# psaegert/bcnf

Hardware: AMD Instinct MI355X
Metric: NLL-training samples/sec + log_prob max-abs-err vs ref, trajectory_FC_small (higher is better)
Workload: dtype f32; 1 GPU; trajectory_FC_small NLL training step (configs[1]); batch_per_gpu=4096, global_batch=4096, parallelism=dp1, hip_graph=True, n_blocks=32, n_conditions=80

## Files before the change

bcnf_amd/csrc/bcnf_stack.hip:

```cpp
#include "bcnf_device.h"
#include "../../include/bcnf_amd.h"

#include <math.h>
#include <stdlib.h>
#include <string.h>

#include <algorithm>
#include <mutex>
#include <utility>
#include <vector>


#ifdef BCNF_PHASE_STAMPS
#define BCNF_STAMPS 1
#else
#define BCNF_STAMPS 0
#endif

namespace {

constexpr int NC16_MAX = 16;
constexpr int TILE = 256;
__host__ __device__ constexpr int tile_slot(int r, int q) { return 4 * r + ((q + (r >> 1)) & 3); }
__host__ __device__ constexpr int tile_ix(int s, int r) { return 4 * tile_slot(r, s & 3) + (s >> 2); }
// ... 514 lines not shown
      r[i] = g4[idx < n4 ? idx : 0];
    }
  }
  __device__ __forceinline__ void store(float* __restrict__ s) const { store_t(s, (int)threadIdx.x); }
  __device__ __forceinline__ void load_t(const float* __restrict__ g, int n, int t) {
    const floatx4* g4 = reinterpret_cast<const floatx4*>(g);
    const int n4 = n >> 2;
#pragma unroll
    for (int i = 0; i < N; ++i) {
      const int idx = t + i * BCNF_WG;
      r[i] = g4[idx < n4 ? idx : 0];
    }
  }
  __device__ __forceinline__ void store_t(float* __restrict__ s, int t) const {
    floatx4* s4 = reinterpret_cast<floatx4*>(s);
#pragma unroll
    for (int i = 0; i < N; ++i) s4[t + i * BCNF_WG] = r[i];
  }
};

constexpr int KC = 128;
constexpr int KCP = KC + 4;
constexpr int BNS = 80;
__host__ __device__ constexpr int bstride16(int n) { return n + ((16 - (n & 31)) & 31); }

template <bool VEC>
__device__ __forceinline__ void load_rows64(const float* __restrict__ M, long long nrows, int ncols, long long ld,
                                            long long r0, int c0, floatx4* reg, int ones = -1) {
#pragma unroll
  for (int e = 0; e < 8; ++e) {
    const int i4 = threadIdx.x + 256 * e, row = i4 >> 5, col = c0 + (i4 & 31) * 4;
    const long long r = r0 + row < nrows ? r0 + row : nrows - 1;
    if (VEC) {
      const floatx4 v = *reinterpret_cast<const floatx4*>(M + r * ld + (col < ncols ? col : 0));
#pragma unroll
      for (int q = 0; q < 4; ++q) reg[e][q] = (r0 + row < nrows && col + q < ncols) ? v[q] : 0.f;
    } else {
#pragma unroll
      for (int q = 0; q < 4; ++q) {
        const int cq = col + q;
        const float v = M[r * ld + (cq < ncols ? cq : ncols - 1)];
        reg[e][q] = (r0 + row < nrows && cq < ncols) ? v : 0.f;
      }
    }
    if (ones >= 0) {
#pragma unroll
      for (int q = 0; q < 4; ++q)
        if (col + q == ones && r0 + row < nrows) reg[e][q] = 1.f;
    }
  }
}

template <bool VEC>
__global__ __launch_bounds__(BCNF_WG) void k_hp(BcnfLayout L, const float* __restrict__ pk,
                                                const float* __restrict__ h, long long R, float* __restrict__ hp) {
  extern __shared__ __attribute__((aligned(16))) float smem[];
  float* As = smem;
  float* Bs = smem + 64 * KCP;
  const int tid = threadIdx.x, wave = tid >> 6, l = tid & 63, lr = l & 15, lq = l >> 4;
  const long long b0 = (long long)blockIdx.x * 64;
  const int n0 = blockIdx.y * 64;
  const int Cp = L.Cp, NKp = L.NKp;
  const float* w1c = pk + L.w1c_off;
  floatx4 ra[8], rb[8];
  auto load = [&](int c0) {
    load_rows64<VEC>(h, R, L.C, L.ldh, b0, c0, ra);
#pragma unroll
    for (int e = 0; e < 8; ++e) {
      const int i4 = tid + 256 * e, row = c0 + (i4 >> 4), col = n0 + (i4 & 15) * 4;
      const floatx4 v = *reinterpret_cast<const floatx4*>(w1c + (long long)(row < Cp ? row : Cp - 1) * NKp + col);
      rb[e] = v * (row < Cp ? 1.f : 0.f);
    }
  };
  auto store = [&]() {
#pragma unroll
    for (int e = 0; e < 8; ++e) {
      const int i4 = tid + 256 * e;
      *reinterpret_cast<floatx4*>(As + (i4 >> 5) * KCP + (i4 & 31) * 4) = ra[e];
      *reinterpret_cast<floatx4*>(Bs + (i4 >> 4) * BNS + (i4 & 15) * 4) = rb[e];
    }
  };
  floatx4 acc[4];
#pragma unroll
  for (int u = 0; u < 4; ++u) acc[u] = floatx4{0.f, 0.f, 0.f, 0.f};
  load(0);
  float b1v[4];
#pragma unroll
  for (int u = 0; u < 4; ++u) b1v[u] = pk[L.b1c_off + n0 + 16 * u + lr];
  for (int c0 = 0; c0 < Cp; c0 += KC) {
    store();
    __syncthreads();
    if (c0 + KC < Cp) load(c0 + KC);
    const int ks = (Cp - c0 < KC ? Cp - c0 : KC) >> 2;
    for (int t0 = 0; t0 < ks; t0 += 4) {
      float a[4], bv[4][4];
#pragma unroll
      for (int t = 0; t < 4; ++t) {
        a[t] = As[(16 * wave + lr) * KCP + 4 * (t0 + t) + lq];
#pragma unroll
        for (int u = 0; u < 4; ++u) bv[t][u] = Bs[(4 * (t0 + t) + lq) * BNS + 16 * u + lr];
      }
#pragma unroll
      for (int t = 0; t < 4; ++t)
#pragma unroll
        for (int u = 0; u < 4; ++u) acc[u] = mfma4(a[t], bv[t][u], acc[u]);
    }
// ... 32 lines not shown
      ra[e] = v * (k < L.nb ? 1.f : 0.f);
    }
#pragma unroll
    for (int e = 0; e < 2; ++e) {
      const int i4 = tid + 256 * e, kj = kj0 + (i4 >> 2);
      const floatx4 v = *reinterpret_cast<const floatx4*>(w1r + (long long)(kj < K ? kj : K - 1) * Cp + (i4 & 3) * 4);
      rb[e] = v * (kj < K ? 1.f : 0.f);
    }
  };
  auto store = [&]() {
#pragma unroll
    for (int e = 0; e < 8; ++e) *reinterpret_cast<floatx4*>(As + arow * KCP + 16 * e + aj4) = ra[e];
#pragma unroll
    for (int e = 0; e < 2; ++e) *reinterpret_cast<floatx4*>(Bs + (tid + 256 * e) * 4) = rb[e];
  };
  floatx4 acc = {0.f, 0.f, 0.f, 0.f}, acc1 = {0.f, 0.f, 0.f, 0.f};
  load(0);
  for (int kj0 = 0; kj0 < K; kj0 += KC) {
    store();
    __syncthreads();
    if (kj0 + KC < K) load(kj0 + KC);
    const int ks = (K - kj0 < KC ? K - kj0 : KC) >> 2;
    for (int t0 = 0; t0 < ks; t0 += 4) {
      float a[4], bv[4];
#pragma unroll
      for (int t = 0; t < 4; ++t) {
        a[t] = As[(16 * wave + lr) * KCP + 4 * (t0 + t) + lq];
        bv[t] = Bs[(4 * (t0 + t) + lq) * 16 + lr];
      }
      acc = mfma4(a[0], bv[0], acc);
      acc1 = mfma4(a[1], bv[1], acc1);
      acc = mfma4(a[2], bv[2], acc);
      acc1 = mfma4(a[3], bv[3], acc1);
    }
    __syncthreads();
  }
  acc += acc1;
  const int col = 16 * n + lr;
  if (col < L.C) {
#pragma unroll
    for (int i = 0; i < 4; ++i) {
      const long long r = b0 + 16 * wave + 4 * lq + i;
      if (r < B) dh[r * L.C + col] = acc[i];
    }
  }
}

__global__ __launch_bounds__(BCNF_WG) void k_dh(BcnfLayout L, const float* __restrict__ pk,
                                                const float* __restrict__ d1, long long B, float* __restrict__ dh) {
  extern __shared__ __attribute__((aligned(16))) float smem[];
  dh_body(L, pk, d1, B, dh, blockIdx.x, blockIdx.y, smem);
}

template <bool VEC, int BPW = 4>
__device__ __forceinline__ void dw1h_body(const BcnfLayout& L, const float* __restrict__ d1, const float* __restrict__ h,
                                          long long B, int rows_per_split, float* __restrict__ work, int bx, int by,
                                          float* __restrict__ smem, int ones = -1) {
  const int hs = bstride16(L.Cp);
  float* As = smem;
  float* Bs = smem + 16 * BPW * KCP;
  const int tid = threadIdx.x, wave = tid >> 6, l = tid & 63, lr = l & 15, lq = l >> 4;
  const int k0 = bx * BPW, s = by;
  const long long m0 = (long long)s * rows_per_split;
  long long m1 = m0 + rows_per_split;
  if (m1 > B) m1 = B;
  const int NC16 = L.Cp >> 4;
  {
    const int row = tid >> 1, j8 = (tid & 1) * 8;
    const long long b = m0 + row;
    const bool ok = b < m1;
    const long long bb = ok ? b : m1 - 1;
    floatx4 va[2 * BPW];
#pragma unroll
    for (int kk = 0; kk < BPW; ++kk) {
      const int k = k0 + kk < L.nb ? k0 + kk : L.nb - 1;
      const floatx4* src = reinterpret_cast<const floatx4*>(d1 + ((long long)k * B + bb) * 16 + j8);
      va[2 * kk] = src[0];
      va[2 * kk + 1] = src[1];
    }
    floatx4 rv[2][8];
#pragma unroll
    for (int half = 0; half < 2; ++half) load_rows64<VEC>(h, m1, L.C, L.ldh, m0 + 64 * half, 0, rv[half], ones);
#pragma unroll
    for (int kk = 0; kk < BPW; ++kk) {
      const float m = (ok && k0 + kk < L.nb) ? 1.f : 0.f;
      const floatx4 v0 = va[2 * kk] * m, v1 = va[2 * kk + 1] * m;
#pragma unroll
      for (int q = 0; q < 4; ++q) {
        As[(kk * 16 + j8 + q) * KCP + row] = v0[q];
        As[(kk * 16 + j8 + 4 + q) * KCP + row] = v1[q];
      }
    }
#pragma unroll
    for (int half = 0; half < 2; ++half) {
#pragma unroll
      for (int e = 0; e < 8; ++e) {
        const int i4 = tid + 256 * e, r = 64 * half + (i4 >> 5), col = (i4 & 31) * 4;
        if (col < L.Cp) *reinterpret_cast<floatx4*>(Bs + r * hs + col) = rv[half][e];
      }
    }
    for (int c0 = KC; c0 < L.Cp; c0 += KC) {
#pragma unroll
      for (int half = 0; half < 2; ++half) {
        load_rows64<VEC>(h, m1, L.C, L.ldh, m0 + 64 * half, c0, rv[half], ones);
#pragma unroll
        for (int e = 0; e < 8; ++e) {
          const int i4 = tid + 256 * e, r = 64 * half + (i4 >> 5), col = c0 + (i4 & 31) * 4;
          if (col < L.Cp) *reinterpret_cast<floatx4*>(Bs + r * hs + col) = rv[half][e];
        }
      }
    }
  }
  __syncthreads();
  const int kw = BPW == 4 ? wave : wave >> 1;
  const int k = k0 + kw;
  const int nh = BPW == 4 ? NC16 : (NC16 + 1) >> 1;
  const int n_lo = BPW == 4 ? 0 : (wave & 1) * nh, n_hi = min(NC16, n_lo + nh);
  float* o = work + (((long long)s * L.nb + (k < L.nb ? k : 0)) * 16) * L.Cp;
  for (int n = n_lo; n < n_hi; ++n) {
    floatx4 acc = {0.f, 0.f, 0.f, 0.f}, acc1 = {0.f, 0.f, 0.f, 0.f};
    for (int t0 = 0; t0 < KC / 4; t0 += 8) {
      float a[8], bv[8];
#pragma unroll
      for (int t = 0; t < 8; ++t) {
        a[t] = As[(16 * kw + lr) * KCP + 4 * (t0 + t) + lq];
        bv[t] = Bs[(4 * (t0 + t) + lq) * hs + 16 * n + lr];
      }
#pragma unroll
      for (int t = 0; t < 8; t += 2) {
        acc = mfma4(a[t], bv[t], acc);
        acc1 = mfma4(a[t + 1], bv[t + 1], acc1);
      }
    }
    acc += acc1;
    if (k < L.nb) {
#pragma unroll
      for (int i = 0; i < 4; ++i) o[(long long)(4 * lq + i) * L.Cp + 16 * n + lr] = acc[i];
    }
  }
}

template <bool VEC>
__global__ __launch_bounds__(BCNF_WG) void k_dw1h(BcnfLayout L, const float* __restrict__ d1,
                                                  const float* __restrict__ h, long long B, int rows_per_split,
                                                  float* __restrict__ work) {
  extern __shared__ __attribute__((aligned(16))) float smem[];
  dw1h_body<VEC>(L, d1, h, B, rows_per_split, work, blockIdx.x, blockIdx.y, smem);
}

size_t hp_lds_bytes() { return sizeof(float) * (size_t)(64 * KCP + KC * BNS); }
size_t dh_lds_bytes() { return sizeof(float) * (size_t)(64 * KCP + KC * 16); }
size_t dw1h_lds_bytes(const BcnfLayout& L, int bpw = 4) {
  return sizeof(float) * (size_t)(16 * bpw * KCP + KC * bstride16(L.Cp));
}

template <bool VEC>
__global__ __launch_bounds__(BCNF_WG) void k_fold_splitk(BcnfLayout F, const float* __restrict__ d1,
                                                         const float* __restrict__ x, long long B, int rows_per_split,
                                                         float* __restrict__ work, int gx_dw, int ones,
                                                         FoldAdamArgs A) {
  extern __shared__ __attribute__((aligned(16))) float smem[];
  if (A.on && blockIdx.x == gridDim.x - 1) {
    if (threadIdx.x == 0) adam_scalars_publish(A);
    return;
  }
  dw1h_body<VEC, 2>(F, d1, x, B, rows_per_split, work, blockIdx.x % gx_dw, blockIdx.x / gx_dw, smem, ones);
}

__global__ __launch_bounds__(BCNF_WG) void k_dw1h_reduce(BcnfLayout L, const float* __restrict__ work, int splits,
                                                         float* __restrict__ dparams) {
  const long long per = 16LL * L.Cp, total = (long long)L.nb * per;
  const long long i = (long long)blockIdx.x * BCNF_WG + threadIdx.x;
  if (i >= total) return;
  const int k = (int)(i / per);
  const int rem = (int)(i - (long long)k * per);
  const int j = rem / L.Cp, c = rem - j * L.Cp;
  if (j >= L.H[1] || c >= L.C) return;
  float acc = 0.f;
  int s = 0;
  for (; s + 8 <= splits; s += 8) {
    float v[8];
#pragma unroll
    for (int t = 0; t < 8; ++t) v[t] = work[(long long)(s + t) * total + i];
#pragma unroll
    for (int t = 0; t < 8; ++t) acc += v[t];
  }
  for (; s < splits; ++s) acc += work[(long long)s * total + i];
  dparams[coupling_base(L, k) + L.lin_w[1] + j * L.lin_in[1] + L.Da + c] = acc;
}

__device__ __forceinline__ void gx_reduce_body(long long total, const float* __restrict__ work, int splits,
                                               float* __restrict__ gx, long long i) {
  if (i >= total) return;
  float acc = 0.f;
  int s = 0;
  for (; s + 16 <= splits; s += 16) {
    float v[16];
#pragma unroll
    for (int t = 0; t < 16; ++t) v[t] = work[(long long)(s + t) * total + i];
#pragma unroll
    for (int t = 0; t < 16; ++t) acc += v[t];
  }
  for (; s < splits; ++s) acc += work[(long long)s * total + i];
  gx[i] = acc;
}

__device__ __forceinline__ int c0_of_finish(int bx, int nct) { return (bx % nct) * 16; }

constexpr int FIN_KC = 512;
constexpr int FIN_SMEM = 2 * FIN_KC * 16;

__device__ __forceinline__ void tile16_accum(const float* __restrict__ As, const float* __restrict__ Bs, int kn,
                                             floatx4 (&acc)[4]) {
  const int lane = threadIdx.x & 63, ks = lane & 15, rb = lane >> 4, cb = threadIdx.x >> 6;
#pragma unroll 4
  for (int k = ks; k < kn; k += 16) {
    const floatx4 a = *reinterpret_cast<const floatx4*>(As + k * 16 + 4 * rb);
    const floatx4 b = *reinterpret_cast<const floatx4*>(Bs + k * 16 + 4 * cb);
#pragma unroll
    for (int r = 0; r < 4; ++r)
#pragma unroll
      for (int c = 0; c < 4; ++c) acc[r][c] = fmaf(a[r], b[c], acc[r][c]);
  }
}

__device__ __forceinline__ float tile16_reduce(float* __restrict__ red, const floatx4 (&acc)[4]) {
  const int lane = threadIdx.x & 63, ks = lane & 15, rb = lane >> 4, cb = threadIdx.x >> 6;
  __syncthreads();
#pragma unroll
  for (int r = 0; r < 4; ++r)
#pragma unroll
    for (int c = 0; c < 4; ++c) red[ks * 256 + (4 * rb + r) * 16 + 4 * cb + c] = acc[r][c];
  __syncthreads();
  float v = 0.f;
#pragma unroll
  for (int q = 0; q < 16; ++q) v += red[q * 256 + threadIdx.x];
  return v;
}

__global__ __launch_bounds__(BCNF_WG) void k_fold_finish(BcnfLayout L, const float* __restrict__ pk,
                                                         const float* __restrict__ gx, const float* __restrict__ wf,
                                                         const float* __restrict__ bf, int X,
                                                         float* __restrict__ dparams, float* __restrict__ dwf,
                                                         float* __restrict__ dbf, FoldAdamArgs A) {
  extern __shared__ __attribute__((aligned(16))) float smem[];
  float* As = smem;
  float* Bs = smem + FIN_KC * 16;
  const int Xp = fold_xp(X), tid = threadIdx.x, nct = L.Cp >> 4;
  floatx4 acc[4];
#pragma unroll
  for (int q = 0; q < 4; ++q) acc[q] = floatx4{0.f, 0.f, 0.f, 0.f};
  const bool adam = A.on && !(A.guard && A.guard[BCNF_GUARD_HALTED]);
  AdamScalars as{};
  const bool keeper = adam && blockIdx.x == 0 && tid == 0;
  const bool logger = keeper && A.log_values && A.log_history;
  long long log_row = 0;
  float step0 = 0.f, log_v[3];
// ... 1410 lines not shown
      }
      gya = an_sa * dxa;
      gyb = an_sb * dxb;
      PHS(1)
      __syncthreads();
      PHS(2)
    }
    if (dy && valid) {
      if (j < Da) dy[b * D + j] = gya;
      if (j < Db) dy[b * D + Da + j] = gyb;
    }
  }
#if BCNF_STAMPS
  if (blockIdx.x == 0 && (threadIdx.x == 0 || threadIdx.x == BCNF_WG))
    for (int i = 0; i < 4; ++i) g_phase[(helper ? 4 : 0) + i] = ph_acc[i];
#endif
#undef PHS
  if (loss_out && blockIdx.x == 0) {
    __syncthreads();
    nll_finalize<BWD_WG>(nll_part, (int)gridDim.x, B, loss_out, rng_w, guard, dT);
  }
}

template <int N>
__device__ __forceinline__ int lpick(const int (&a)[N], int i) {
  int r = a[0];
#pragma unroll
  for (int t = 1; t < N; ++t) r = (i == t) ? a[t] : r;
  return r;
}

__device__ __forceinline__ long long slab_to_canonical(const BcnfLayout& L, int m, int o) {
  const int NH = L.NH, NW = NH + 2;
  const int cb = m * L.blk_stride + ((m < L.nb - 1) ? L.an_size : 0);
  if (o < NW * 256) {
    const int c = o >> 8, e = o & 255, lane = e >> 2;
    const int row = 4 * (lane >> 4) + (e & 3), col = lane & 15;
    const int l = c < NH ? c + 1 : NH + 1;
    const int nrows = c < NH ? lpick(L.H, l) : L.Db, ncols = (l == 1) ? L.Da : lpick(L.H, l - 1);
    if (row >= nrows || col >= ncols) return -1;
    const int row0 = (c == NH + 1) ? L.Db : 0;
    return (long long)cb + lpick(L.lin_w, l) + (row0 + row) * lpick(L.lin_in, l) + col;
  }
  const int o2 = o - NW * 256, c = o2 >> 4, r = o2 & 15;
  if (c < NH) return r < lpick(L.H, c + 1) ? (long long)cb + lpick(L.lin_b, c + 1) + r : -1;
  if (c < NH + 2) return r < L.Db ? (long long)cb + lpick(L.lin_b, NH + 1) + ((c == NH + 1) ? L.Db : 0) + r : -1;
  const int a = c - NH - 2;
  if (a >= 4 || !L.act_norm || m >= L.nb - 1 || r >= ((a < 2) ? L.Da : L.Db)) return -1;
  return (long long)m * L.blk_stride + ((a & 1) ? L.D : 0) + ((a < 2) ? 0 : L.Da) + r;
}

constexpr int RED_G = 8, RED_O4 = 32, RED_T = 16;

__device__ __forceinline__ void reduce_body(const BcnfLayout& L, const float* __restrict__ slab, long long stride,
                                            int nwg, float* __restrict__ out, int bx, float* __restrict__ smem,
                                            const FoldAdamArgs* A = nullptr, const AdamScalars* as = nullptr) {
  floatx4 (*part)[RED_O4] = reinterpret_cast<floatx4 (*)[RED_O4]>(smem);
  const int g = threadIdx.x / RED_O4, o4 = threadIdx.x % RED_O4;
  const long long i = ((long long)bx * RED_O4 + o4) * 4;
  const bool live = i < stride;
  const long long ic = live ? i : 0;
  const int m = (int)(ic / L.sblk), o = (int)(ic - (long long)m * L.sblk);
  long long ci[4];
  float ap[4], am[4], av[4];
#pragma unroll
  for (int e = 0; e < 4; ++e) {
    ci[e] = slab_to_canonical(L, m, o + e);
    if (A && g == 0) {
      const long long c = ci[e] >= 0 ? ci[e] : 0;
      ap[e] = A->p[0][c];
      am[e] = A->m[0][c];
      av[e] = A->v[0][c];
    }
  }
  floatx4 acc = {0.f, 0.f, 0.f, 0.f};
  int w = g;
  for (; w + RED_G * (RED_T - 1) < nwg; w += RED_G * RED_T) {
    floatx4 v[RED_T];
#pragma unroll
    for (int t = 0; t < RED_T; ++t)
      v[t] = *reinterpret_cast<const floatx4*>(slab + (long long)(w + RED_G * t) * stride + ic);
#pragma unroll
    for (int t = 0; t < RED_T; ++t) acc += v[t];
  }
  for (; w < nwg; w += RED_G) acc += *reinterpret_cast<const floatx4*>(slab + (long long)w * stride + ic);
  part[g][o4] = acc;
  __syncthreads();
  if (g != 0 || !live) return;
  floatx4 tot = part[0][o4];
#pragma unroll
  for (int q = 1; q < RED_G; ++q) tot += part[q][o4];
#pragma unroll
  for (int e = 0; e < 4; ++e) {
    if (ci[e] < 0) continue;
    out[ci[e]] = tot[e];
    if (A) {
      adam_elem(ap[e], tot[e], am[e], av[e], *as);
      A->p[0][ci[e]] = ap[e];
      A->m[0][ci[e]] = am[e];
      A->v[0][ci[e]] = av[e];
    }
  }
}

struct TailGrid {
  int n_dh, gx_dh;
  int n_red;
  int gx_dw;
  int ones;
};

template <bool VEC>
__global__ __launch_bounds__(BCNF_WG) void k_bwd_tail(BcnfLayout L, BcnfLayout Lw, TailGrid G, const float* __restrict__ pk,
                                                      const float* __restrict__ d1, const float* __restrict__ h,
                                                      long long B, float* __restrict__ dh,
                                                      const float* __restrict__ slab, long long stride, int nwg,
                                                      float* __restrict__ dparams, int rows_per_split,
                                                      float* __restrict__ work) {
  extern __shared__ __attribute__((aligned(16))) float smem[];
  int i = blockIdx.x;
  if (i < G.n_dh) {
    dh_body(L, pk, d1, B, dh, i % G.gx_dh, i / G.gx_dh, smem);
    return;
  }
  i -= G.n_dh;
  if (i < G.n_red) {
    reduce_body(L, slab, stride, nwg, dparams, i, smem);
    return;
  }
  i -= G.n_red;
  dw1h_body<VEC>(Lw, d1, h, B, rows_per_split, work, i % G.gx_dw, i / G.gx_dw, smem, G.ones);
}

__global__ __launch_bounds__(BCNF_WG) void k_red_gx(BcnfLayout L, long long total, const float* __restrict__ work,
                                                    int splits, float* __restrict__ gx, int n_gx,
                                                    const float* __restrict__ slab, long long stride, int nwg,
                                                    float* __restrict__ dparams, FoldAdamArgs A) {
  __shared__ __attribute__((aligned(16))) float smem[RED_G * RED_O4 * 4];
  const int bx = blockIdx.x;
  if (bx < n_gx) {
    gx_reduce_body(total, work, splits, gx, (long long)bx * BCNF_WG + threadIdx.x);
    return;
  }
  if (A.on && !(A.guard && A.guard[BCNF_GUARD_HALTED])) {
    const AdamScalars as = adam_scalars_of(A, A.asc[0], A.asc[1]);
    reduce_body(L, slab, stride, nwg, dparams, bx - n_gx, smem, &A, &as);
    return;
  }
  reduce_body(L, slab, stride, nwg, dparams, bx - n_gx, smem);
}

__global__ __launch_bounds__(BCNF_WG) void k_fill_lds(float value) {
  extern __shared__ __attribute__((aligned(16))) float smem[];
  for (int i = threadIdx.x; i < (int)(LDS_MAX / 16); i += BCNF_WG)
    reinterpret_cast<floatx4*>(smem)[i] = floatx4{value, value, value, value};
  __syncthreads();
}

int check_launch() { return bcnf_rt::launched(); }



std::mutex g_attr_mu;
const void* g_attr_fn[256];
size_t g_attr_lds[256];
int g_attr_n = 0;

template <typename K>
int launch_lds(K kernel, size_t& lds) {
  if (lds > LDS_MAX) return BCNF_ERR_UNSUPPORTED;
  const void* fn = reinterpret_cast<const void*>(kernel);
  std::lock_guard<std::mutex> lk(g_attr_mu);
  for (int i = 0; i < g_attr_n; ++i)
    if (g_attr_fn[i] == fn && g_attr_lds[i] >= lds) return BCNF_OK;
  const hipError_t e = hipFuncSetAttribute(fn, hipFuncAttributeMaxDynamicSharedMemorySize, (int)lds);
  if (e != hipSuccess) return bcnf_rt::hip_status(e);
  int slot = -1;
  for (int i = 0; i < g_attr_n; ++i)
    if (g_attr_fn[i] == fn) slot = i;
  if (slot < 0 && g_attr_n < 256) slot = g_attr_n++;
  if (slot >= 0) {
    g_attr_fn[slot] = fn;
    g_attr_lds[slot] = lds;
  }
  return BCNF_OK;
}

template <int NH>
bool layout_matches(const BcnfLayout& L) {
  return L.rf_b1 == RecF<NH>::B1 && L.rf_w1 == RecF<NH>::W1 && L.rf_hid == RecF<NH>::HID && L.rf_t == RecF<NH>::T &&
         L.rf_s == RecF<NH>::S && L.rf_q == RecF<NH>::Q && L.RF >= RecF<NH>::USED && L.rb_w1t == RecB<NH>::W1T &&
         L.rb_hid == RecB<NH>::HID && L.rb_tt == RecB<NH>::TT && L.rb_st == RecB<NH>::ST && L.rb_qt == RecB<NH>::QT &&
         L.rb_an == RecB<NH>::AN && L.RB >= RecB<NH>::USED;
}

struct NllOut {
  float* part = nullptr;
};

bool vec_rows(const BcnfLayout& L, const float* h) { return L.ldh % 4 == 0 && ((uintptr_t)h & 15) == 0; }

int launch_hp(const BcnfLayout& L, const float* pk, const float* h, long long R, float* hp, hipStream_t st) {
// ... 208 lines not shown
}

int bcnf_stack_forward(const BcnfStackDesc* desc, const void* packed, const float* y, const float* h, int64_t batch,
                       float* z, float* ldj, float* log_prob, int32_t training, const uint64_t* rng_state,
                       void* workspace, int32_t save, void* stream) {
  return forward_impl(desc, packed, y, h, batch, z, ldj, log_prob, training, rng_state, workspace, save != 0, false,
                      false, nullptr, nullptr, stream);
}

int bcnf_nll_forward(const BcnfStackDesc* desc, const void* packed, const float* y, const float* h, int64_t batch,
                     float* z, float* ldj, int32_t training, uint64_t* rng_state, void* workspace, int32_t finalize,
                     float* loss_out, int32_t* guard, void* stream) {
  return forward_impl(desc, packed, y, h, batch, z, ldj, nullptr, training, rng_state, workspace, true, true,
                      finalize != 0, loss_out, guard, stream);
}

int bcnf_stack_backward(const BcnfStackDesc* desc, const void* packed, const float* h, const float* dz,
                        const float* dldj, int64_t batch, int32_t training, void* workspace, float* dy,
                        float* dh, float* dparams, void* slab, void* stream) {
  return backward_impl(desc, packed, h, dz, dldj, nullptr, 0, batch, training, workspace, dy, dh, dparams, slab,
                       nullptr, nullptr, nullptr, stream);
}

int bcnf_nll_backward(const BcnfStackDesc* desc, const void* packed, const float* h, const float* z,
                      const float* dloss, int64_t batch, int32_t training, void* workspace, float* dy,
                      float* dh, float* dparams, void* slab, float* loss_out, uint64_t* rng_state, int32_t* guard,
                      void* stream) {
  if (!z && batch > 0) return BCNF_ERR_ARG;
  return backward_impl(desc, packed, h, z, nullptr, dloss, 1, batch, training, workspace, dy, dh, dparams, slab,
                       loss_out, rng_state, guard, stream);
}

int bcnf_backward_tail(const BcnfStackDesc* desc, const void* packed, const void* slab, const float* h,
                       const void* workspace, int64_t batch, int32_t training, float* dh, float* dparams,
                       void* stream) {
  BcnfLayout L;
  int rc = make_layout(desc, &L);
  if (rc) return rc;
  if (!layout_supported(L, desc)) return BCNF_ERR_UNSUPPORTED;
  if (!packed || !slab || !h || !workspace || !dparams || batch < 1) return BCNF_ERR_ARG;
  hipStream_t st = (hipStream_t)stream;
  const long long S = slab_stride_of(L);
  const int nwg = (int)((batch + 15) / 16);
  const bool drop = training && L.p > 0.f;
  const float* d1 = (const float*)workspace + ws_d1_off(L, batch, drop);
  float* work = (float*)slab + (long long)nwg * S;
  const int rps = w1h_rows_per_split(batch);
  const long long splits = w1h_splits(batch);
  TailGrid G;
  G.gx_dh = (int)((batch + 63) / 64);
  G.n_dh = dh ? G.gx_dh * (L.Cp >> 4) : 0;
  G.n_red = (int)((S / 4 + RED_O4 - 1) / RED_O4);
  G.gx_dw = (L.nb + 3) / 4;
  G.ones = -1;
  const long long n_dw = (long long)G.gx_dw * splits;
  size_t lds = dw1h_lds_bytes(L);
  if (dh_lds_bytes() > lds) lds = dh_lds_bytes();
  const dim3 grid((unsigned)(G.n_dh + G.n_red + n_dw));
  if (vec_rows(L, h)) {
    if ((rc = launch_lds(k_bwd_tail<true>, lds))) return rc;
    hipLaunchKernelGGL(k_bwd_tail<true>, grid, dim3(BCNF_WG), lds, st, L, L, G, (const float*)packed, d1, h,
                       (long long)batch, dh, (const float*)slab, S, nwg, dparams, rps, work);
  } else {
    if ((rc = launch_lds(k_bwd_tail<false>, lds))) return rc;
    hipLaunchKernelGGL(k_bwd_tail<false>, grid, dim3(BCNF_WG), lds, st, L, L, G, (const float*)packed, d1, h,
                       (long long)batch, dh, (const float*)slab, S, nwg, dparams, rps, work);
  }
  if ((rc = check_launch())) return rc;
  const long long outs = (long long)L.nb * 16 * L.Cp;
  hipLaunchKernelGGL(k_dw1h_reduce, dim3((unsigned)((outs + BCNF_WG - 1) / BCNF_WG)), dim3(BCNF_WG), 0, st, L,
                     (const float*)work, (int)splits, dparams);
  return check_launch();
}

namespace {
int fold_setup(const BcnfStackDesc* desc, int32_t X, BcnfLayout* L) {
  int rc = make_layout(desc, L);
  if (rc) return rc;
  if (!layout_supported(*L, desc)) return BCNF_ERR_UNSUPPORTED;
  if (X < 1 || fold_xp(X) > 16 * NC16_MAX) return BCNF_ERR_UNSUPPORTED;
  if (dw1h_lds_bytes(fold_layout(*L, X, X)) > LDS_MAX) return BCNF_ERR_UNSUPPORTED;
  return BCNF_OK;
}
long long fold_floats(const BcnfLayout& L, int X) { return (long long)(fold_xp(X) + 1) * L.NKp; }
bool raw_applicable(const BcnfLayout& L, int X) {
  return X <= RAW_KP - 4 && L.C <= 64 * RAW_TPW && L.nb >= 2 && L.act_norm;
}
}

int bcnf_fold_bytes(const BcnfStackDesc* desc, int32_t in_features, int64_t* bytes) {
  BcnfLayout L;
  const int rc = fold_setup(desc, in_features, &L);
  if (rc) return rc;
  if (!bytes) return BCNF_ERR_ARG;
  *bytes = fold_floats(L, in_features) * 4;
  return BCNF_OK;
}

int bcnf_fold_slab_bytes(const BcnfStackDesc* desc, int32_t in_features, int64_t batch, int64_t* bytes) {
  BcnfLayout L;
  const int rc = fold_setup(desc, in_features, &L);
  if (rc) return rc;
  if (!bytes || batch < 0) return BCNF_ERR_ARG;
  const BcnfLayout F = fold_layout(L, in_features, in_features);
  *bytes = ((int64_t)((batch + 15) / 16) * slab_stride_of(L) + w1h_work_floats(F, batch) +
            (int64_t)L.nb * 16 * F.Cp + 4) * 4;
  return BCNF_OK;
}

int bcnf_pack_params_fold(const BcnfStackDesc* desc, const float* params, const float* qmats,
                          const float* feat_weight, const float* feat_bias, int32_t in_features, void* packed,
                          float* fold, const BcnfGather2* gather, void* stream) {
  BcnfLayout L;
  int rc = fold_setup(desc, in_features, &L);
  if (rc) return rc;
  if (!params || !packed || !fold || !feat_weight || (L.nb > 1 && !qmats)) return BCNF_ERR_ARG;
  BcnfGatherArgs ga = {};
  if (gather) {
    const BcnfGather2& g = *gather;
    if (g.n < 1 || g.cols0 < 1 || g.cols1 < 1 || !g.idx || !g.src0 || !g.dst0 || !g.src1 || !g.dst1)
      return BCNF_ERR_ARG;
    if (g.n * (int64_t)(g.cols0 + g.cols1) >= (1LL << 31)) return BCNF_ERR_UNSUPPORTED;
    ga = BcnfGatherArgs{g.idx, (const long long*)g.cursor, g.src0, g.dst0, g.src1, g.dst1, (int)g.n, 0, g.cols0,
                        g.cols1, 0};
    gather2_plan(g.n, &ga.rpw, &ga.nwg);
  }
  const int npw = pack_wgs(L, true);
  const unsigned grid = (unsigned)(L.NKp / 16 * FOLD_SPLIT + ga.nwg + npw + 1);
  hipLaunchKernelGGL(k_pack_fold, dim3(grid), dim3(BCNF_WG), 0, (hipStream_t)stream, L, params, qmats, (float*)packed,
                     feat_weight, feat_bias, (int)in_features, fold, ga, npw);
  return check_launch();
}

int bcnf_fold_nll_forward(const BcnfStackDesc* desc, const void* packed, const float* fold, int32_t in_features,
                          const float* y, const float* x, int32_t ldx, int64_t batch, float* z, float* ldj, int32_t training,
                          uint64_t* rng_state, void* workspace, int32_t finalize, float* loss_out, int32_t* guard,
                          void* stream) {
  BcnfLayout L;
  const int rc = fold_setup(desc, in_features, &L);
  if (rc) return rc;
  if (!fold || ldx < in_features) return BCNF_ERR_ARG;
  return forward_impl(desc, packed, y, x, batch, z, ldj, nullptr, training, rng_state, workspace, true, true,
                      finalize != 0, loss_out, guard, stream, fold, in_features, ldx);
}

int bcnf_lds_fill(float value, void* stream) {
  size_t lds = LDS_MAX;
  const int rc = launch_lds(k_fill_lds, lds);
  if (rc) return rc;
  hipLaunchKernelGGL(k_fill_lds, dim3(4 * 256), dim3(BCNF_WG), LDS_MAX, (hipStream_t)stream, value);
  return check_launch();
}

int bcnf_fold_raw_table_bytes(const BcnfStackDesc* desc, int32_t in_features, int64_t* bytes) {
  BcnfLayout L;
  const int rc = fold_setup(desc, in_features, &L);
  if (rc) return rc;
  if (!bytes) return BCNF_ERR_ARG;
  if (!raw_applicable(L, in_features)) return BCNF_ERR_UNSUPPORTED;
// ... 49 lines not shown
    R.ldx = ldx;
  }
  return forward_impl(desc, packed, R.ypool, R.xpool, batch, z, ldj, nullptr, training, rng_state, workspace, true,
                      true, finalize != 0, loss_out, guard, stream, nullptr, 0, 0, &R);
}

int bcnf_fold_backward_tail(const BcnfStackDesc* desc, const void* packed, const void* slab, const float* x,
                            int32_t ldx, int32_t in_features, const float* feat_weight, const float* feat_bias,
                            const void* workspace, int64_t batch, int32_t training, float* dparams,
                            float* dfeat_weight, float* dfeat_bias, const BcnfFoldAdam* adam, void* stream) {
  BcnfLayout L;
  int rc = fold_setup(desc, in_features, &L);
  if (rc) return rc;
  if (!packed || !slab || !x || !feat_weight || !workspace || !dparams || batch < 1 || ldx < in_features)
    return BCNF_ERR_ARG;
  FoldAdamArgs A = {};
  if (adam) {
    const BcnfFoldAdam& a = *adam;
    if (!a.params[0] || !a.exp_avg[0] || !a.exp_avg_sq[0] || !a.params[1] || !a.exp_avg[1] || !a.exp_avg_sq[1] ||
        !a.step || !a.done_counter || (feat_bias && (!a.params[2] || !a.exp_avg[2] || !a.exp_avg_sq[2])) ||
        (a.advance_cursor && a.cursor_modulo < 1))
      return BCNF_ERR_ARG;
    for (int t = 0; t < 3; ++t) {
      A.p[t] = a.params[t];
      A.m[t] = a.exp_avg[t];
      A.v[t] = a.exp_avg_sq[t];
    }
    if (!feat_bias) A.p[2] = A.m[2] = A.v[2] = nullptr;
    A.step = a.step;
    A.lr = a.lr;
    A.b1 = a.beta1;
    A.b2 = a.beta2;
    A.eps = a.eps;
    A.wd = a.weight_decay;
    A.cursor = (long long*)a.advance_cursor;
    A.n_batches = (long long)a.cursor_modulo;
    A.log_values = a.log_values;
    A.log_history = a.log_history;
    A.done = (int*)a.done_counter;
    A.guard = (const int*)a.guard;
    A.on = 1;
  }
  const BcnfLayout F = fold_layout(L, in_features, ldx);
  hipStream_t st = (hipStream_t)stream;
  const long long S = slab_stride_of(L);
  const int nwg = (int)((batch + 15) / 16);
  const bool drop = training && L.p > 0.f;
  const float* d1 = (const float*)workspace + ws_d1_off(L, batch, drop);
  float* work = (float*)slab + (long long)nwg * S;
  float* gx = work + w1h_work_floats(F, batch);
  A.asc = gx + (long long)L.nb * 16 * F.Cp;
  const int rps = w1h_rows_per_split(batch);
  const long long splits = w1h_splits(batch);
  const int n_red = (int)((S / 4 + RED_O4 - 1) / RED_O4);
  const int gx_dw = (L.nb + 1) / 2;
  const dim3 grid((unsigned)((long long)gx_dw * splits + (A.on ? 1 : 0)));
  size_t lds = dw1h_lds_bytes(F, 2);
  if (vec_rows(F, x)) {
    if ((rc = launch_lds(k_fold_splitk<true>, lds))) return rc;
    hipLaunchKernelGGL(k_fold_splitk<true>, grid, dim3(BCNF_WG), lds, st, F, d1, x, (long long)batch, rps, work, gx_dw,
                       (int)in_features, A);
  } else {
    if ((rc = launch_lds(k_fold_splitk<false>, lds))) return rc;
    hipLaunchKernelGGL(k_fold_splitk<false>, grid, dim3(BCNF_WG), lds, st, F, d1, x, (long long)batch, rps, work, gx_dw,
                       (int)in_features, A);
  }
  if ((rc = check_launch())) return rc;
  const long long total = (long long)L.nb * 16 * F.Cp;
  const int n_gx = (int)((total + BCNF_WG - 1) / BCNF_WG);
  hipLaunchKernelGGL(k_red_gx, dim3((unsigned)(n_gx + n_red)), dim3(BCNF_WG), 0, st, L, total, (const float*)work,
                     (int)splits, gx, n_gx, (const float*)slab, S, nwg, dparams, A);
  if ((rc = check_launch())) return rc;
  const int n_fin = (L.nb + (F.Cp >> 4)) * (L.Cp >> 4);
  size_t fin_lds = sizeof(float) * FIN_SMEM;
  if ((rc = launch_lds(k_fold_finish, fin_lds))) return rc;
  hipLaunchKernelGGL(k_fold_finish, dim3((unsigned)n_fin), dim3(BCNF_WG), fin_lds, st, L, (const float*)packed,
                     (const float*)gx, feat_weight, feat_bias, (int)in_features, dparams, dfeat_weight, dfeat_bias, A);
  return check_launch();
}

int bcnf_grad_reduce(const BcnfStackDesc* desc, const void* slab, const float* h, const void* workspace,
                     int64_t batch, int32_t training, float* dparams, void* stream) {
  return bcnf_backward_tail(desc, slab, slab, h, workspace, batch, training, nullptr, dparams, stream);
}

int bcnf_stack_dh(const BcnfStackDesc* desc, const void* packed, const void* workspace, int64_t batch, int32_t training,
                  float* dh, void* stream) {
  BcnfLayout L;
  int rc = make_layout(desc, &L);
  if (rc) return rc;
  if (!layout_supported(L, desc)) return BCNF_ERR_UNSUPPORTED;
  if (batch < 0 || !packed || !workspace || !dh) return BCNF_ERR_ARG;
  if (batch == 0) return BCNF_OK;
  const float* d1 = (const float*)workspace + ws_d1_off(L, batch, training && L.p > 0.f);
  size_t lds = dh_lds_bytes();
  if ((rc = launch_lds(k_dh, lds))) return rc;
  hipLaunchKernelGGL(k_dh, dim3((unsigned)((batch + 63) / 64), (unsigned)(L.Cp >> 4)), dim3(BCNF_WG), lds,
                     (hipStream_t)stream, L, (const float*)packed, d1, (long long)batch, dh);
  return check_launch();
}

int bcnf_stack_inverse(const BcnfStackDesc* desc, const void* packed, const float* z, const float* h, int64_t h_rows,
                       const int64_t* cond_index, int64_t n_rows, float* y, int32_t training,
                       const uint64_t* rng_state, void* scratch, void* stream) {
  BcnfLayout L;
  int rc = make_layout(desc, &L);
  if (rc) return rc;
  if (!layout_supported(L, desc)) return BCNF_ERR_UNSUPPORTED;
  if (n_rows == 0) return BCNF_OK;
  if (n_rows < 0 || h_rows < 1 || !packed || !z || !h || !y || !scratch) return BCNF_ERR_ARG;
  if (!cond_index && h_rows != n_rows) return BCNF_ERR_ARG;
  const bool drop = training && L.p > 0.f;
  if (drop && !rng_state) return BCNF_ERR_ARG;
  const float* pk = (const float*)packed;
  hipStream_t st = (hipStream_t)stream;
  float* hp = (float*)scratch;
  if ((rc = launch_hp(L, pk, h, h_rows, hp, st))) return rc;
  switch (L.NH) {
#define BCNF_CASE(N) case N: return inv_dispatch<N>(L, pk, z, hp, h_rows, cond_index, n_rows, y, drop, rng_state, st);
    BCNF_CASE(1) BCNF_CASE(2) BCNF_CASE(3) BCNF_CASE(4) BCNF_CASE(5) BCNF_CASE(6) BCNF_CASE(7) BCNF_CASE(8)
#undef BCNF_CASE
    default: return BCNF_ERR_UNSUPPORTED;
  }
}

const char* bcnf_status_string(int status) {
  switch (status) {
    case BCNF_OK: return "ok";
    case BCNF_ERR_ARG: return "invalid argument";
    case BCNF_ERR_UNSUPPORTED: return "unsupported stack shape for the fused kernel family";
// ... 52 lines not shown
```

Before: 30.22 million samples/s.

## Fuse fold split-K with slab reduce and stage fold weights in one tail kernel

After: 31.23 million samples/s (median of 6 runs). 1.03x the previous value.

```diff
diff --git a/bcnf_amd/csrc/bcnf_stack.hip b/bcnf_amd/csrc/bcnf_stack.hip
--- a/bcnf_amd/csrc/bcnf_stack.hip
+++ b/bcnf_amd/csrc/bcnf_stack.hip
@@ -590,6 +590,34 @@
 }
 
 template <bool VEC>
+__device__ __forceinline__ void rows64_issue(const float* __restrict__ M, long long nrows, int ncols, long long ld,
+                                             long long r0, int c0, floatx4* reg) {
+#pragma unroll
+  for (int e = 0; e < 8; ++e) {
+    const int i4 = threadIdx.x + 256 * e, row = i4 >> 5, col = c0 + (i4 & 31) * 4;
+    const long long r = r0 + row < nrows ? r0 + row : nrows - 1;
+    if (VEC) {
+      reg[e] = *reinterpret_cast<const floatx4*>(M + r * ld + (col < ncols ? col : 0));
+    } else {
+#pragma unroll
+      for (int q = 0; q < 4; ++q) reg[e][q] = M[r * ld + (col + q < ncols ? col + q : ncols - 1)];
+    }
+  }
+}
+__device__ __forceinline__ void rows64_mask(long long nrows, int ncols, long long r0, int c0, floatx4* reg, int ones) {
+#pragma unroll
+  for (int e = 0; e < 8; ++e) {
+    const int i4 = threadIdx.x + 256 * e, row = i4 >> 5, col = c0 + (i4 & 31) * 4;
+    const bool in = r0 + row < nrows;
+#pragma unroll
+    for (int q = 0; q < 4; ++q) {
+      const float v = (in && col + q < ncols) ? reg[e][q] : 0.f;
+      reg[e][q] = (in && col + q == ones) ? 1.f : v;
+    }
+  }
+}
+
+template <bool VEC>
 __global__ __launch_bounds__(BCNF_WG) void k_hp(BcnfLayout L, const float* __restrict__ pk,
                                                 const float* __restrict__ h, long long R, float* __restrict__ hp) {
   extern __shared__ __attribute__((aligned(16))) float smem[];
@@ -728,15 +756,15 @@
   dh_body(L, pk, d1, B, dh, blockIdx.x, blockIdx.y, smem);
 }
 
-template <bool VEC, int BPW = 4>
+template <bool VEC>
 __device__ __forceinline__ void dw1h_body(const BcnfLayout& L, const float* __restrict__ d1, const float* __restrict__ h,
                                           long long B, int rows_per_split, float* __restrict__ work, int bx, int by,
-                                          float* __restrict__ smem, int ones = -1) {
+                                          float* __restrict__ smem) {
   const int hs = bstride16(L.Cp);
   float* As = smem;
-  float* Bs = smem + 16 * BPW * KCP;
+  float* Bs = smem + 64 * KCP;
   const int tid = threadIdx.x, wave = tid >> 6, l = tid & 63, lr = l & 15, lq = l >> 4;
-  const int k0 = bx * BPW, s = by;
+  const int k0 = bx * 4, s = by;
   const long long m0 = (long long)s * rows_per_split;
   long long m1 = m0 + rows_per_split;
   if (m1 > B) m1 = B;
@@ -746,9 +774,9 @@
     const long long b = m0 + row;
     const bool ok = b < m1;
     const long long bb = ok ? b : m1 - 1;
-    floatx4 va[2 * BPW];
-#pragma unroll
-    for (int kk = 0; kk < BPW; ++kk) {
+    floatx4 va[8];
+#pragma unroll
+    for (int kk = 0; kk < 4; ++kk) {
       const int k = k0 + kk < L.nb ? k0 + kk : L.nb - 1;
       const floatx4* src = reinterpret_cast<const floatx4*>(d1 + ((long long)k * B + bb) * 16 + j8);
       va[2 * kk] = src[0];
@@ -756,9 +784,9 @@
     }
     floatx4 rv[2][8];
 #pragma unroll
-    for (int half = 0; half < 2; ++half) load_rows64<VEC>(h, m1, L.C, L.ldh, m0 + 64 * half, 0, rv[half], ones);
-#pragma unroll
-    for (int kk = 0; kk < BPW; ++kk) {
+    for (int half = 0; half < 2; ++half) load_rows64<VEC>(h, m1, L.C, L.ldh, m0 + 64 * half, 0, rv[half]);
+#pragma unroll
+    for (int kk = 0; kk < 4; ++kk) {
       const float m = (ok && k0 + kk < L.nb) ? 1.f : 0.f;
       const floatx4 v0 = va[2 * kk] * m, v1 = va[2 * kk + 1] * m;
 #pragma unroll
@@ -778,7 +806,7 @@
     for (int c0 = KC; c0 < L.Cp; c0 += KC) {
 #pragma unroll
       for (int half = 0; half < 2; ++half) {
-        load_rows64<VEC>(h, m1, L.C, L.ldh, m0 + 64 * half, c0, rv[half], ones);
+        load_rows64<VEC>(h, m1, L.C, L.ldh, m0 + 64 * half, c0, rv[half]);
 #pragma unroll
         for (int e = 0; e < 8; ++e) {
           const int i4 = tid + 256 * e, r = 64 * half + (i4 >> 5), col = c0 + (i4 & 31) * 4;
@@ -788,18 +816,15 @@
     }
   }
   __syncthreads();
-  const int kw = BPW == 4 ? wave : wave >> 1;
-  const int k = k0 + kw;
-  const int nh = BPW == 4 ? NC16 : (NC16 + 1) >> 1;
-  const int n_lo = BPW == 4 ? 0 : (wave & 1) * nh, n_hi = min(NC16, n_lo + nh);
+  const int k = k0 + wave;
   float* o = work + (((long long)s * L.nb + (k < L.nb ? k : 0)) * 16) * L.Cp;
-  for (int n = n_lo; n < n_hi; ++n) {
+  for (int n = 0; n < NC16; ++n) {
     floatx4 acc = {0.f, 0.f, 0.f, 0.f}, acc1 = {0.f, 0.f, 0.f, 0.f};
     for (int t0 = 0; t0 < KC / 4; t0 += 8) {
       float a[8], bv[8];
 #pragma unroll
       for (int t = 0; t < 8; ++t) {
-        a[t] = As[(16 * kw + lr) * KCP + 4 * (t0 + t) + lq];
+        a[t] = As[(16 * wave + lr) * KCP + 4 * (t0 + t) + lq];
         bv[t] = Bs[(4 * (t0 + t) + lq) * hs + 16 * n + lr];
       }
 #pragma unroll
@@ -826,21 +851,102 @@
 
 size_t hp_lds_bytes() { return sizeof(float) * (size_t)(64 * KCP + KC * BNS); }
 size_t dh_lds_bytes() { return sizeof(float) * (size_t)(64 * KCP + KC * 16); }
-size_t dw1h_lds_bytes(const BcnfLayout& L, int bpw = 4) {
-  return sizeof(float) * (size_t)(16 * bpw * KCP + KC * bstride16(L.Cp));
-}
-
-template <bool VEC>
-__global__ __launch_bounds__(BCNF_WG) void k_fold_splitk(BcnfLayout F, const float* __restrict__ d1,
-                                                         const float* __restrict__ x, long long B, int rows_per_split,
-                                                         float* __restrict__ work, int gx_dw, int ones,
-                                                         FoldAdamArgs A) {
-  extern __shared__ __attribute__((aligned(16))) float smem[];
-  if (A.on && blockIdx.x == gridDim.x - 1) {
-    if (threadIdx.x == 0) adam_scalars_publish(A);
-    return;
-  }
-  dw1h_body<VEC, 2>(F, d1, x, B, rows_per_split, work, blockIdx.x % gx_dw, blockIdx.x / gx_dw, smem, ones);
+size_t dw1h_lds_bytes(const BcnfLayout& L) { return sizeof(float) * (size_t)(64 * KCP + KC * bstride16(L.Cp)); }
+
+constexpr int KH = KC / 2, KHP = KH + 4;
+template <bool VEC, int NT>
+__device__ __forceinline__ void dw1h_half_body(const BcnfLayout& L, const float* __restrict__ d1,
+                                               const float* __restrict__ h, long long B, int rows_per_split,
+                                               float* __restrict__ work, int bx, int by, float* __restrict__ smem,
+                                               int ones) {
+  const int hs = bstride16(L.Cp);
+  float* As = smem;
+  float* Bs = smem + 32 * KHP;
+  const int tid = threadIdx.x, wave = tid >> 6, l = tid & 63, lr = l & 15, lq = l >> 4;
+  const int k0 = bx * 2, s = by;
+  const long long m0 = (long long)s * rows_per_split;
+  long long m1 = m0 + rows_per_split;
+  if (m1 > B) m1 = B;
+  const int NC16 = L.Cp >> 4;
+  const int row = tid >> 2, j4 = (tid & 3) * 4;
+  floatx4 va[2], rv[8];
+  float am[2];
+  auto load_half = [&](int half) {
+    rows64_issue<VEC>(h, m1, L.C, L.ldh, m0 + KH * half, 0, rv);
+    const long long b = m0 + KH * half + row;
+    const bool ok = b < m1;
+    const long long bb = ok ? b : m1 - 1;
+#pragma unroll
+    for (int kk = 0; kk < 2; ++kk) {
+      const int k = k0 + kk < L.nb ? k0 + kk : L.nb - 1;
+      va[kk] = *reinterpret_cast<const floatx4*>(d1 + ((long long)k * B + bb) * 16 + j4);
+      am[kk] = (ok && k0 + kk < L.nb) ? 1.f : 0.f;
+    }
+  };
+  const int kw = wave >> 1, k = k0 + kw;
+  const int nh = (NC16 + 1) >> 1, n_lo = (wave & 1) * nh, n_hi = min(NC16, n_lo + nh);
+  floatx4 acc[NT], acc1[NT];
+#pragma unroll
+  for (int j = 0; j < NT; ++j) acc[j] = acc1[j] = floatx4{0.f, 0.f, 0.f, 0.f};
+#pragma unroll
+  for (int half = 0; half < 2; ++half) {
+    load_half(half);
+    if (half) __syncthreads();
+    rows64_mask(m1, L.C, m0 + KH * half, 0, rv, ones);
+#pragma unroll
+    for (int e = 0; e < 8; ++e) {
+      const int i4 = tid + 256 * e, r = i4 >> 5, col = (i4 & 31) * 4;
+      if (col < L.Cp) *reinterpret_cast<floatx4*>(Bs + r * hs + col) = rv[e];
+    }
+#pragma unroll
+    for (int kk = 0; kk < 2; ++kk) {
+      const floatx4 v = va[kk] * am[kk];
+#pragma unroll
+      for (int q = 0; q < 4; ++q) As[(kk * 16 + j4 + q) * KHP + row] = v[q];
+    }
+    for (int c0 = KC; c0 < L.Cp; c0 += KC) {
+      rows64_issue<VEC>(h, m1, L.C, L.ldh, m0 + KH * half, c0, rv);
+      rows64_mask(m1, L.C, m0 + KH * half, c0, rv, ones);
+#pragma unroll
+      for (int e = 0; e < 8; ++e) {
+        const int i4 = tid + 256 * e, r = i4 >> 5, col = c0 + (i4 & 31) * 4;
+        if (col < L.Cp) *reinterpret_cast<floatx4*>(Bs + r * hs + col) = rv[e];
+      }
+    }
+    __syncthreads();
+#pragma unroll
+    for (int j = 0; j < NT; ++j) {
+      const int n = n_lo + j;
+      if (n >= n_hi) continue;
+#pragma unroll
+      for (int t0 = 0; t0 < KH / 4; t0 += 8) {
+        float a[8], bv[8];
+#pragma unroll
+        for (int t = 0; t < 8; ++t) {
+          a[t] = As[(16 * kw + lr) * KHP + 4 * (t0 + t) + lq];
+          bv[t] = Bs[(4 * (t0 + t) + lq) * hs + 16 * n + lr];
+        }
+#pragma unroll
+        for (int t = 0; t < 8; t += 2) {
+          acc[j] = mfma4(a[t], bv[t], acc[j]);
+          acc1[j] = mfma4(a[t + 1], bv[t + 1], acc1[j]);
+        }
+      }
+    }
+  }
+  if (k >= L.nb) return;
+  float* o = work + (((long long)s * L.nb + k) * 16) * L.Cp;
+#pragma unroll
+  for (int j = 0; j < NT; ++j) {
+    const int n = n_lo + j;
+    if (n >= n_hi) continue;
+    const floatx4 r = acc[j] + acc1[j];
+#pragma unroll
+    for (int i = 0; i < 4; ++i) o[(long long)(4 * lq + i) * L.Cp + 16 * n + lr] = r[i];
+  }
+}
+size_t dw1h_half_lds_bytes(const BcnfLayout& L) {
+  return sizeof(float) * (size_t)(32 * KHP + KH * bstride16(L.Cp));
 }
 
 __global__ __launch_bounds__(BCNF_WG) void k_dw1h_reduce(BcnfLayout L, const float* __restrict__ work, int splits,
@@ -879,6 +985,11 @@
   }
   for (; s < splits; ++s) acc += work[(long long)s * total + i];
   gx[i] = acc;
+}
+
+__global__ __launch_bounds__(BCNF_WG) void k_fold_gx(long long total, const float* __restrict__ work, int splits,
+                                                     float* __restrict__ gx) {
+  gx_reduce_body(total, work, splits, gx, (long long)blockIdx.x * BCNF_WG + threadIdx.x);
 }
 
 __device__ __forceinline__ int c0_of_finish(int bx, int nct) { return (bx % nct) * 16; }
@@ -2395,10 +2506,13 @@
 
 constexpr int RED_G = 8, RED_O4 = 32, RED_T = 16;
 
+constexpr int RED_SMEM = RED_G * RED_O4 * 4 + 4;
+
 __device__ __forceinline__ void reduce_body(const BcnfLayout& L, const float* __restrict__ slab, long long stride,
                                             int nwg, float* __restrict__ out, int bx, float* __restrict__ smem,
-                                            const FoldAdamArgs* A = nullptr, const AdamScalars* as = nullptr) {
+                                            const FoldAdamArgs* A = nullptr) {
   floatx4 (*part)[RED_O4] = reinterpret_cast<floatx4 (*)[RED_O4]>(smem);
+  float* sc = smem + RED_G * RED_O4 * 4;
   const int g = threadIdx.x / RED_O4, o4 = threadIdx.x % RED_O4;
   const long long i = ((long long)bx * RED_O4 + o4) * 4;
   const bool live = i < stride;
@@ -2406,6 +2520,7 @@
   const int m = (int)(ic / L.sblk), o = (int)(ic - (long long)m * L.sblk);
   long long ci[4];
   float ap[4], am[4], av[4];
+  const float step0 = A ? A->step[0] : 0.f;
 #pragma unroll
   for (int e = 0; e < 4; ++e) {
     ci[e] = slab_to_canonical(L, m, o + e);
@@ -2416,6 +2531,13 @@
       av[e] = A->v[0][c];
     }
   }
+  bool scalars_due = A != nullptr;
+  auto scalars = [&]() {
+    const double t = (double)(step0 + 1.0f);
+    if (threadIdx.x == 0) sc[0] = (float)(A->lr / (1.0 - pow(A->b1, t)));
+    if (threadIdx.x == 64) sc[1] = (float)sqrt(1.0 - pow(A->b2, t));
+    scalars_due = false;
+  };
   floatx4 acc = {0.f, 0.f, 0.f, 0.f};
   int w = g;
   for (; w + RED_G * (RED_T - 1) < nwg; w += RED_G * RED_T) {
@@ -2423,22 +2545,26 @@
 #pragma unroll
     for (int t = 0; t < RED_T; ++t)
       v[t] = *reinterpret_cast<const floatx4*>(slab + (long long)(w + RED_G * t) * stride + ic);
+    if (scalars_due) scalars();
 #pragma unroll
     for (int t = 0; t < RED_T; ++t) acc += v[t];
   }
   for (; w < nwg; w += RED_G) acc += *reinterpret_cast<const floatx4*>(slab + (long long)w * stride + ic);
+  if (scalars_due) scalars();
   part[g][o4] = acc;
   __syncthreads();
   if (g != 0 || !live) return;
   floatx4 tot = part[0][o4];
 #pragma unroll
   for (int q = 1; q < RED_G; ++q) tot += part[q][o4];
+  AdamScalars as{};
+  if (A) as = adam_scalars_of(*A, sc[0], sc[1]);
 #pragma unroll
   for (int e = 0; e < 4; ++e) {
     if (ci[e] < 0) continue;
     out[ci[e]] = tot[e];
     if (A) {
-      adam_elem(ap[e], tot[e], am[e], av[e], *as);
+      adam_elem(ap[e], tot[e], am[e], av[e], as);
       A->p[0][ci[e]] = ap[e];
       A->m[0][ci[e]] = am[e];
       A->v[0][ci[e]] = av[e];
@@ -2450,11 +2576,10 @@
   int n_dh, gx_dh;
   int n_red;
   int gx_dw;
-  int ones;
 };
 
 template <bool VEC>
-__global__ __launch_bounds__(BCNF_WG) void k_bwd_tail(BcnfLayout L, BcnfLayout Lw, TailGrid G, const float* __restrict__ pk,
+__global__ __launch_bounds__(BCNF_WG) void k_bwd_tail(BcnfLayout L, TailGrid G, const float* __restrict__ pk,
                                                       const float* __restrict__ d1, const float* __restrict__ h,
                                                       long long B, float* __restrict__ dh,
                                                       const float* __restrict__ slab, long long stride, int nwg,
@@ -2472,25 +2597,46 @@
     return;
   }
   i -= G.n_red;
-  dw1h_body<VEC>(Lw, d1, h, B, rows_per_split, work, i % G.gx_dw, i / G.gx_dw, smem, G.ones);
-}
-
-__global__ __launch_bounds__(BCNF_WG) void k_red_gx(BcnfLayout L, long long total, const float* __restrict__ work,
-                                                    int splits, float* __restrict__ gx, int n_gx,
-                                                    const float* __restrict__ slab, long long stride, int nwg,
-                                                    float* __restrict__ dparams, FoldAdamArgs A) {
-  __shared__ __attribute__((aligned(16))) float smem[RED_G * RED_O4 * 4];
+  dw1h_body<VEC>(L, d1, h, B, rows_per_split, work, i % G.gx_dw, i / G.gx_dw, smem);
+}
+
+template <bool VEC, int NT>
+__global__ __launch_bounds__(BCNF_WG, VEC && NT <= 3 ? 4 : 2) void k_fold_tail(BcnfLayout L, BcnfLayout F, const float* __restrict__ d1,
+                                                       const float* __restrict__ x, long long B, int rows_per_split,
+                                                       float* __restrict__ work, int gx_dw, int n_sk, int ones,
+                                                       const float* __restrict__ slab, long long stride, int nwg,
+                                                       float* __restrict__ dparams, const float* __restrict__ wf,
+                                                       const float* __restrict__ bf, float* __restrict__ wf1,
+                                                       FoldAdamArgs A) {
+  extern __shared__ __attribute__((aligned(16))) float smem[];
   const int bx = blockIdx.x;
-  if (bx < n_gx) {
-    gx_reduce_body(total, work, splits, gx, (long long)bx * BCNF_WG + threadIdx.x);
+  if (bx < n_sk) {
+    dw1h_half_body<VEC, NT>(F, d1, x, B, rows_per_split, work, bx % gx_dw, bx / gx_dw, smem, ones);
     return;
   }
+  if (bx == n_sk) {
+    const int nw = L.C * F.C, n1 = nw + (bf ? L.C : 0);
+    for (int i0 = 0; i0 < n1; i0 += 16 * BCNF_WG) {
+      float v[16];
+#pragma unroll
+      for (int e = 0; e < 16; ++e) {
+        const int i = min(i0 + e * BCNF_WG + (int)threadIdx.x, n1 - 1);
+        v[e] = i < nw ? wf[i] : bf[i - nw];
+      }
+#pragma unroll
+      for (int e = 0; e < 16; ++e) {
+        const int i = i0 + e * BCNF_WG + (int)threadIdx.x;
+        if (i < n1) wf1[i] = v[e];
+      }
+    }
+    if (A.on && threadIdx.x == 0) adam_scalars_publish(A);
+    return;
+  }
   if (A.on && !(A.guard && A.guard[BCNF_GUARD_HALTED])) {
-    const AdamScalars as = adam_scalars_of(A, A.asc[0], A.asc[1]);
-    reduce_body(L, slab, stride, nwg, dparams, bx - n_gx, smem, &A, &as);
+    reduce_body(L, slab, stride, nwg, dparams, bx - n_sk - 1, smem, &A);
     return;
   }
-  reduce_body(L, slab, stride, nwg, dparams, bx - n_gx, smem);
+  reduce_body(L, slab, stride, nwg, dparams, bx - n_sk - 1, smem);
 }
 
 __global__ __launch_bounds__(BCNF_WG) void k_fill_lds(float value) {
@@ -2805,18 +2951,17 @@
   G.n_dh = dh ? G.gx_dh * (L.Cp >> 4) : 0;
   G.n_red = (int)((S / 4 + RED_O4 - 1) / RED_O4);
   G.gx_dw = (L.nb + 3) / 4;
-  G.ones = -1;
   const long long n_dw = (long long)G.gx_dw * splits;
   size_t lds = dw1h_lds_bytes(L);
   if (dh_lds_bytes() > lds) lds = dh_lds_bytes();
   const dim3 grid((unsigned)(G.n_dh + G.n_red + n_dw));
   if (vec_rows(L, h)) {
     if ((rc = launch_lds(k_bwd_tail<true>, lds))) return rc;
-    hipLaunchKernelGGL(k_bwd_tail<true>, grid, dim3(BCNF_WG), lds, st, L, L, G, (const float*)packed, d1, h,
+    hipLaunchKernelGGL(k_bwd_tail<true>, grid, dim3(BCNF_WG), lds, st, L, G, (const float*)packed, d1, h,
                        (long long)batch, dh, (const float*)slab, S, nwg, dparams, rps, work);
   } else {
     if ((rc = launch_lds(k_bwd_tail<false>, lds))) return rc;
-    hipLaunchKernelGGL(k_bwd_tail<false>, grid, dim3(BCNF_WG), lds, st, L, L, G, (const float*)packed, d1, h,
+    hipLaunchKernelGGL(k_bwd_tail<false>, grid, dim3(BCNF_WG), lds, st, L, G, (const float*)packed, d1, h,
                        (long long)batch, dh, (const float*)slab, S, nwg, dparams, rps, work);
   }
   if ((rc = check_launch())) return rc;
@@ -2857,7 +3002,8 @@
   if (!bytes || batch < 0) return BCNF_ERR_ARG;
   const BcnfLayout F = fold_layout(L, in_features, in_features);
   *bytes = ((int64_t)((batch + 15) / 16) * slab_stride_of(L) + w1h_work_floats(F, batch) +
-            (int64_t)L.nb * 16 * F.Cp + 4) * 4;
+            (int64_t)L.nb * 16 * F.Cp + 4 +
+            (int64_t)L.C * (in_features + 1)) * 4;
   return BCNF_OK;
 }
 
@@ -3013,30 +3159,38 @@
   A.asc = gx + (long long)L.nb * 16 * F.Cp;
   const int rps = w1h_rows_per_split(batch);
   const long long splits = w1h_splits(batch);
+  float* wf1 = A.asc + 4;
+  const float* bf1 = feat_bias ? wf1 + (long long)L.C * in_features : nullptr;
   const int n_red = (int)((S / 4 + RED_O4 - 1) / RED_O4);
   const int gx_dw = (L.nb + 1) / 2;
-  const dim3 grid((unsigned)((long long)gx_dw * splits + (A.on ? 1 : 0)));
-  size_t lds = dw1h_lds_bytes(F, 2);
-  if (vec_rows(F, x)) {
-    if ((rc = launch_lds(k_fold_splitk<true>, lds))) return rc;
-    hipLaunchKernelGGL(k_fold_splitk<true>, grid, dim3(BCNF_WG), lds, st, F, d1, x, (long long)batch, rps, work, gx_dw,
-                       (int)in_features, A);
-  } else {
-    if ((rc = launch_lds(k_fold_splitk<false>, lds))) return rc;
-    hipLaunchKernelGGL(k_fold_splitk<false>, grid, dim3(BCNF_WG), lds, st, F, d1, x, (long long)batch, rps, work, gx_dw,
-                       (int)in_features, A);
-  }
+  const long long n_sk = (long long)gx_dw * splits;
+  const dim3 grid((unsigned)(n_sk + 1 + n_red));
+  size_t lds = dw1h_half_lds_bytes(F);
+  if (lds < sizeof(float) * RED_SMEM) lds = sizeof(float) * RED_SMEM;
+  const bool vec = vec_rows(F, x);
+  const bool nt3 = (F.Cp >> 4) <= 6;
+#define BCNF_FOLD_TAIL(V, NT)                                                                                      \
+  do {                                                                                                             \
+    if ((rc = launch_lds(k_fold_tail<V, NT>, lds))) return rc;                                                     \
+    hipLaunchKernelGGL((k_fold_tail<V, NT>), grid, dim3(BCNF_WG), lds, st, L, F, d1, x, (long long)batch, rps, work, \
+                       gx_dw, (int)n_sk, (int)in_features, (const float*)slab, S, nwg, dparams, feat_weight,       \
+                       feat_bias, wf1, A);                                                                         \
+  } while (0)
+  if (vec && nt3) BCNF_FOLD_TAIL(true, 3);
+  else if (vec) BCNF_FOLD_TAIL(true, 8);
+  else if (nt3) BCNF_FOLD_TAIL(false, 3);
+  else BCNF_FOLD_TAIL(false, 8);
+#undef BCNF_FOLD_TAIL
   if ((rc = check_launch())) return rc;
   const long long total = (long long)L.nb * 16 * F.Cp;
-  const int n_gx = (int)((total + BCNF_WG - 1) / BCNF_WG);
-  hipLaunchKernelGGL(k_red_gx, dim3((unsigned)(n_gx + n_red)), dim3(BCNF_WG), 0, st, L, total, (const float*)work,
-                     (int)splits, gx, n_gx, (const float*)slab, S, nwg, dparams, A);
+  hipLaunchKernelGGL(k_fold_gx, dim3((unsigned)((total + BCNF_WG - 1) / BCNF_WG)), dim3(BCNF_WG), 0, st, total,
+                     (const float*)work, (int)splits, gx);
   if ((rc = check_launch())) return rc;
   const int n_fin = (L.nb + (F.Cp >> 4)) * (L.Cp >> 4);
   size_t fin_lds = sizeof(float) * FIN_SMEM;
   if ((rc = launch_lds(k_fold_finish, fin_lds))) return rc;
   hipLaunchKernelGGL(k_fold_finish, dim3((unsigned)n_fin), dim3(BCNF_WG), fin_lds, st, L, (const float*)packed,
-                     (const float*)gx, feat_weight, feat_bias, (int)in_features, dparams, dfeat_weight, dfeat_bias, A);
+                     (const float*)gx, (const float*)wf1, bf1, (int)in_features, dparams, dfeat_weight, dfeat_bias, A);
   return check_launch();
 }
 
```
